# adaly/gridnext

Hardware: AMD Instinct MI355X
Metric: spots/sec training throughput (multimodal f+g) (higher is better)
Workload: dtype f32; 1 GPU; C4: multimodal f(DenseNet-121 @128px + count-MLP 2000 genes) + hex g on 78x64 Visium grids, 1 array (4992 spots) per GPU per step, f frozen/eval (tutorial mode), g trained with Adam, masked CE; spots_per_array=4992, parallelism=dp1

## Files before the change

### gridnext_amd/_lib.py

```python
import ctypes
import os

import torch

_HERE = os.path.dirname(os.path.abspath(__file__))
LIB_PATH = os.environ.get('GNX_LIB') or os.path.join(_HERE, 'libgridnext_hip.so')

_P, _I, _L, _F, _D = ctypes.c_void_p, ctypes.c_int, ctypes.c_long, ctypes.c_float, ctypes.c_double
_LL = ctypes.c_longlong

SIGNATURES = {
    'gnx_hexconv_fwd': (_I, [_P, _P, _P, _P, _P, _I, _I, _I, _I, _I, _I, _P]),
    'gnx_hexconv_bwd_data': (_I, [_P, _P, _P, _P, _I, _I, _I, _I, _I, _I, _P]),
    'gnx_hexconv_bwd_weight_workspace': (_L, [_I, _I, _I, _I, _I]),
    'gnx_hexconv_bwd_weight': (_I, [_P, _P, _P, _P, _P, _P, _I, _I, _I, _I, _I, _I, _I, _P]),
    'gnx_hexconv_bwd_weight_batch': (_I, [_P, _I, _P]),
    'gnx_hexconv_k_fwd': (_I, [_P, _P, _P, _P, _I, _I, _I, _I, _I, _I, _I, _P]),
    'gnx_hexconv_k_bwd_data': (_I, [_P, _P, _P, _I, _I, _I, _I, _I, _I, _I, _P]),
    'gnx_hexconv_k_bwd_weight_workspace': (_L, [_I, _I, _I, _I, _I, _I]),
    'gnx_hexconv_k_bwd_weight': (_I, [_P, _P, _P, _P, _P, _I, _I, _I, _I, _I, _I, _I, _I, _P]),
    'gnx_gridconv_fwd': (_I, [_P, _P, _P, _P, _I, _I, _I, _I, _I, _I, _I, _P]),
    'gnx_gridconv_bwd_data': (_I, [_P, _P, _P, _I, _I, _I, _I, _I, _I, _I, _P]),
    'gnx_gridconv_bwd_weight_workspace': (_L, [_I, _I, _I, _I, _I, _I, _I]),
    'gnx_gridconv_bwd_weight': (_I, [_P, _P, _P, _P, _P, _I, _I, _I, _I, _I, _I, _I, _I, _P]),
# ... 50 lines not shown
    'gnx_conv_stem_bnrelu_maxpool_h16': (_I, [_P, _P, _P, _L, _L, _I, _I, _I, _I, _I, _I, _I, _I, _P, _P, _P]),
    'gnx_conv_stem_bnrelu_maxpool_u8': (_I, [_P, _P, _P, _L, _L, _I, _I, _I, _I, _I, _I, _I, _I, _P, _P, _P, _I, _P]),
    'gnx_conv_stem_bnrelu_maxpool_f16mul': (_I, [_P, _I, _P, _P, _L, _L, _I, _I, _I, _I, _I, _I, _I, _I, _P, _P, _P, _P]),
    'gnx_u8_to_f32': (_I, [_P, _P, _L, _I, _I, _I, _P, _P]),
    'gnx_resize_ksize': (_I, [_I, _I]),
    'gnx_resize_crop_u8': (_I, [_P, _P, _L, _I, _I, _I, _I, _I, _I, _I, _I, _P, _P, _P, _P, _P]),
    'gnx_resize_crop_u8_f32': (_I, [_P, _P, _L, _I, _I, _I, _I, _I, _I, _I, _I, _P, _P, _P, _P, _P, _P]),
    'gnx_wsi_patch_grid_u8': (_I, [_P, _I, _I, _P, _I, _I, _I, _I, _I, _P, _P, _I, _P, _P]),
    'gnx_wsi_patch_grid_u8_f32': (_I, [_P, _I, _I, _P, _I, _I, _I, _I, _I, _P, _P, _I, _P, _P, _P]),
    'gnx_conv1x1_bnrelu_f16_h': (_I, [_P, _L, _P, _P, _L, _L, _I, _I, _P, _P, _P, _P, _I, _I, _P]),
    'gnx_conv1x1_bnrelu_h16': (_I, [_P, _L, _P, _P, _L, _L, _I, _I, _P, _P, _P, _P, _P]),
    'gnx_bnrelu_avgpool2_h16': (_I, [_P, _L, _P, _L, _L, _I, _I, _P, _P, _P]),
    'gnx_conv3x3_f16_dma_h': (_I, [_P, _L, _P, _P, _L, _L, _I, _I, _I, _P]),
    'gnx_bnrelu_avgpool_h16': (_I, [_P, _L, _P, _L, _L, _I, _I, _P, _P, _P]),
    'gnx_wgrad1x1_f16_workspace': (_L, [_L, _I, _I]),
    'gnx_wgrad1x1_f16': (_I, [_P, _L, _P, _L, _P, _P, _P, _P, _L, _I, _I, _P, _I, _P, _P]),
    'gnx_wgrad3x3_f16_workspace': (_L, [_L]),
    'gnx_wgrad3x3_f16': (_I, [_P, _L, _P, _P, _P, _L, _I, _P, _I, _P, _P]),
    'gnx_conv3x3_dgrad_bnrelu_bwd_f16_workspace': (_L, [_L]),
    'gnx_conv3x3_dgrad_bnrelu_bwd_f16': (_I, [_P, _L, _P, _P, _P, _L, _I, _P, _P, _P, _P, _P, _P, _P, _I, _P, _P]),
    'gnx_conv1x1_dgrad_bnrelu_bwd_f16_workspace': (_L, [_L, _I]),
    'gnx_conv1x1_dgrad_bnrelu_bwd_f16': (_I, [_P, _P, _P, _L, _P, _L, _L, _I, _P, _P, _P, _P, _P, _P, _P, _P, _I, _P, _P]),
    'gnx_conv1x1_dgrad_wgrad_f16_workspace': (_L, [_L, _I]),
    'gnx_conv1x1_dgrad_wgrad_bnrelu_bwd_f16': (_I, [_P, _P, _P, _L, _P, _L, _L, _I, _P, _P, _P, _P, _P, _P, _P, _P, _P, _I, _P, _P]),
    'gnx_tail_bwd_f16_workspace': (_L, [_L, _I]),
    'gnx_tail_bwd_f16': (_I, [_P, _L, _P, _L, _P, _L, _L, _I, _I, _P, _P, _P, _P, _P, _P, _P, _P, _I, _P, _P]),
    'gnx_trans_bwd_f16_workspace': (_L, [_L, _I, _I]),
    'gnx_trans_bwd_f16': (_I, [_P, _L, _P, _L, _P, _L, _L, _I, _I, _P, _P, _P, _P, _P, _P, _P, _P, _I, _P, _P]),
    'gnx_h16_cols_to_f32': (_I, [_P, _L, _P, _L, _L, _I, _P, _P, _P]),
    'gnx_stem_bwd_f16_workspace': (_L, [_L, _I]),
    'gnx_stem_bwd_f16': (_I, [_P, _P, _P, _P, _P, _P, _P, _L, _P, _P, _P, _P, _L, _I, _I, _P, _I, _P, _P]),
    'gnx_dense_layer_f16_pack': (_I, [_P, _P, _P, _P, _I, _P]),
    'gnx_dense_layer_f16': (_I, [_P, _L, _L, _I, _I, _P, _P, _P, _P, _P, _P, _P]),
    'gnx_dense_layer_f16_tape': (_I, [_P, _L, _L, _I, _I, _P, _P, _P, _P, _P, _P, _P, _L, _P]),
    'gnx_dense_bwd_f16_pack': (_I, [_P, _P, _P, _P, _I, _P]),
    'gnx_wgrad3x3_f16_lb': (_I, [_P, _L, _P, _L, _L, _P, _P, _L, _I, _P, _I, _P, _P]),
    'gnx_conv3x3_dgrad_bnrelu_bwd_f16_lb': (_I, [_P, _L, _P, _P, _L, _L, _P, _L, _I, _P, _P, _P, _P, _P, _P, _P, _I, _P, _P]),
    'gnx_conv3x3_bwd_f16_workspace': (_L, [_L]),
    'gnx_conv3x3_bwd_f16_lb': (_I, [_P, _L, _P, _P, _L, _L, _P, _P, _L, _I, _P, _P, _P, _P, _P, _P, _P, _I, _P, _P]),
    'gnx_conv1x1_dgrad_wgrad_bnrelu_bwd_f16_lb': (_I, [_P, _P, _P, _L, _L, _P, _L, _L, _L, _I, _P, _P, _P, _P, _P, _P, _P, _P, _P, _I,
                                                       _P, _P]),
    'gnx_tail_bwd_f16_lb': (_I, [_P, _L, _P, _L, _L, _P, _L, _L, _L, _I, _I, _P, _P, _P, _P, _P, _P, _P, _P, _I, _P, _P]),
    'gnx_trans_bwd_f16_lb': (_I, [_P, _L, _L, _P, _L, _L, _P, _L, _L, _L, _I, _I, _P, _P, _P, _P, _P, _P, _P, _P, _I, _P, _P]),
    'gnx_conv_stem_bnrelu_maxpool_f16mul_cb': (_I, [_P, _I, _P, _P, _L, _L, _I, _I, _I, _I, _I, _I, _I, _I, _P, _P, _P, _P]),
    'gnx_conv1x1_bnrelu_h16_cb': (_I, [_P, _L, _P, _P, _L, _L, _I, _I, _P, _P, _P, _P, _P]),
    'gnx_bnrelu_avgpool2_h16_cb': (_I, [_P, _L, _P, _L, _L, _I, _I, _P, _P, _P]),
    'gnx_transition_f16_pack': (_I, [_P, _P, _I, _I, _P]),
    'gnx_transition_f16': (_I, [_P, _L, _L, _I, _I, _I, _P, _P, _P, _P, _L, _P]),
    'gnx_transition_f16_tape': (_I, [_P, _L, _L, _I, _I, _I, _P, _P, _P, _P, _L, _P, _L, _P]),
    'gnx_bnrelu_avgpool_h16_cb': (_I, [_P, _L, _P, _L, _L, _I, _I, _P, _P, _P]),
    'gnx_conv3x3_bnrelu': (_I, [_P, _L, _P, _P, _L, _L, _I, _I, _I, _P, _P, _P]),
    'gnx_winograd_conv3x3_weights': (_I, [_P, _P, _I, _I, _P]),
    'gnx_conv3x3_winograd': (_I, [_P, _L, _P, _P, _L, _L, _I, _I, _I, _P]),
    'gnx_conv3x3_form': (_I, [_P, _L, _P, _P, _L, _L, _I, _I, _I, _P, _P, _P]),
    'gnx_conv3x3_winograd_form': (_I, [_P, _L, _P, _P, _L, _L, _I, _I, _I, _P]),
    'gnx_conv3x3_dgrad_bnrelu_bwd_form': (_I, [_P, _L, _P, _P, _L, _P, _L, _L, _I, _I, _I, _P, _P, _P, _P, _P, _P]),
    'gnx_conv3x3_f16_dma_form': (_I, [_P, _L, _P, _P, _L, _L, _I, _I, _I, _P]),
    'gnx_conv_stem': (_I, [_P, _P, _P, _L, _L, _I, _I, _I, _I, _I, _I, _I, _I, _P]),
    'gnx_conv_stem_bnrelu_maxpool': (_I, [_P, _P, _P, _L, _L, _I, _I, _I, _I, _I, _I, _I, _I, _P, _P, _P]),
    'gnx_conv_stem_bnrelu_maxpool_argmax': (_I, [_P, _P, _P, _L, _P, _L, _I, _I, _I, _I, _I, _I, _I, _I, _P, _P, _P]),
    'gnx_bnrelu_maxpool': (_I, [_P, _L, _P, _L, _L, _I, _I, _I, _P, _P, _P]),
    'gnx_bnrelu_avgpool': (_I, [_P, _L, _P, _L, _L, _I, _I, _P, _P, _P]),
    'gnx_spot_compact': (_I, [_P, _L, _L, _P, _P, _P, _P, _P]),
    'gnx_spot_broadcast_rows': (_I, [_P, _L, _L, _I, _P, _L, _P]),
    'gnx_conv_stem_bnrelu_maxpool_idx': (_I, [_P, _P, _P, _L, _L, _I, _I, _I, _I, _I, _I, _I, _I, _P, _P, _P, _L, _P]),
    'gnx_conv_stem_bnrelu_maxpool_u8_idx': (_I, [_P, _P, _P, _L, _L, _I, _I, _I, _I, _I, _I, _I, _I, _P, _P, _P, _P, _L, _P]),
    'gnx_bnrelu_avgpool_idx': (_I, [_P, _L, _P, _L, _L, _I, _I, _P, _P, _P, _L, _P]),
    'gnx_wgrad_workspace': (_L, [_L, _I, _I, _I]),
    'gnx_wgrad_bnrelu': (_I, [_P, _L, _P, _L, _P, _P, _P, _P, _L, _I, _I, _I, _I, _I, _I, _P]),
    'gnx_wgrad_bnrelu_batch': (_I, [_P, _I, _I, _P]),
    'gnx_transpose_weight': (_I, [_P, _P, _I, _I, _P]),
    'gnx_relayout_weights_batch': (_I, [_P, _I, _I, _P]),
    'gnx_repack_conv3x3_bwd': (_I, [_P, _P, _I, _I, _P]),
    'gnx_rows_broadcast': (_I, [_P, _L, _P, _L, _L, _I, _I, _F, _P]),
    'gnx_avgpool2_bwd': (_I, [_P, _L, _P, _L, _L, _I, _I, _P]),
    'gnx_maxpool_bwd': (_I, [_P, _L, _P, _L, _P, _L, _P, _L, _L, _I, _I, _I, _P, _P, _P]),
    'gnx_bnrelu_maxpool_argmax': (_I, [_P, _L, _P, _L, _P, _L, _I, _I, _I, _P, _P, _P]),
    'gnx_maxpool_bwd_argmax': (_I, [_P, _P, _L, _P, _L, _L, _I, _I, _I, _P]),
    'gnx_maxpool_bwd_argmax_bnrelu': (_I, [_P, _P, _L, _P, _L, _P, _P, _L, _L, _I, _I, _I, _P]),
    'gnx_conv0_wgrad_workspace': (_L, [_L, _I, _I, _I, _I, _I, _I, _I]),
    'gnx_conv0_wgrad': (_I, [_P, _P, _L, _P, _P, _L, _I, _I, _I, _I, _I, _I, _I, _I, _P]),
    'gnx_conv0_dgrad': (_I, [_P, _L, _P, _P, _L, _I, _I, _I, _I, _I, _I, _I, _P]),
    'gnx_softmax_rows': (_I, [_P, _L, _L, _I, _P, _L, _P, _P]),
    'gnx_gemm_f32': (_I, [_P, _L, _I, _P, _L, _I, _P, _P, _L, _L, _L, _L, _I, _P]),
    'gnx_gemm_f32_workspace': (_L, [_L, _L, _L]),
    'gnx_gemm_f32_ws': (_I, [_P, _L, _I, _P, _L, _I, _P, _P, _L, _L, _L, _L, _I, _P, _P]),
    'gnx_fingerprint128_split_bytes': (_L, []),
    'gnx_fingerprint128_batch_workspace': (_L, [ctypes.c_size_t, _I]),
    'gnx_fingerprint128_batch': (_I, [_P, ctypes.c_size_t, _I, _P, _P, _P]),
    'gnx_rgb_hist_u8_workspace': (_L, [ctypes.c_size_t]),
    'gnx_rgb_hist_u8': (_I, [_P, ctypes.c_size_t, _P, _P, _P]),
    'gnx_rgb_lut_u8': (_I, [_P, _P, ctypes.c_size_t, _P, _P]),
}

_lib = None
_ERRORS = {-1: 'bad argument', -2: 'kernel launch failed', -3: 'unsupported shape'}
ERR_UNSUPPORTED = -3


class HipExtensionMissing(RuntimeError):
    pass


def lib():
    global _lib
    if _lib is None:
# ... 45 lines not shown
```

### gridnext_amd/csrc/conv3x3.hip

```cpp
#include "fwd_common.h"

namespace {

constexpr int C3_BM = 128, C3_BN = 32;

__global__ __launch_bounds__(256) void conv3x3_kernel(const float* __restrict__ A, long lda,
                                                      const float* __restrict__ Wr, float* __restrict__ out, long ldc,
                                                      long M, int N, int K, int S, const float* __restrict__ scale,
                                                      const float* __restrict__ shift, int vecA, int vecW) {
    extern __shared__ __attribute__((aligned(16))) float lds[];
    const int strip = C3_BM + 2 * S + 2;
    float* As = lds;
    float* Bs = lds + strip * LDK;
    const int t = threadIdx.x, lane = t & 63, wave = t >> 6, h = lane >> 5, i = lane & 31;
    const long P0 = (long)blockIdx.x * C3_BM;
    const long base = P0 - S - 1;
    const int n0 = blockIdx.y * C3_BN;
    const bool has_act = scale != nullptr;

    const long P = P0 + 32 * wave + i;
    unsigned mask = 0;
    if (P < M) {
        const int rem = (int)(P % ((long)S * S));
        const int y = rem / S, x = rem - y * S;
// ... 439 lines not shown
        if constexpr (!NK1) store16(0, std::integral_constant<int, 0>{});
    }
    asm volatile("s_waitcnt vmcnt(0)" ::: "memory");
    if constexpr (BNADJ) {
#pragma unroll
        for (int ct = 0; ct < 4; ++ct) {
            const float sb = adj_b[ct] + __shfl_xor(adj_b[ct], 32), sg = adj_g[ct] + __shfl_xor(adj_g[ct], 32);
            if (h == 0) {
                float* sl = bn.slab + (long)(blockIdx.x * NW + wave) * 2 * N + 32 * ct + i;
                sl[0] = sb;
                sl[N] = sg;
            }
        }
    }
}

constexpr int C3_ADJ_LANES = 16;
__global__ __launch_bounds__(64 * C3_ADJ_LANES) void c3_adj_reduce_kernel(const float* __restrict__ slab, int nblk, int C,
                                                                          float* __restrict__ dbeta,
                                                                          float* __restrict__ dgamma, int accumulate) {
    __shared__ float part[C3_ADJ_LANES][64];
    const int cl = threadIdx.x & 63, rl = threadIdx.x >> 6;
    const int idx = blockIdx.x * 64 + cl;
    float s0 = 0.f;
    if (idx < 2 * C) {
        const int q = idx / C, c = idx - q * C;
        const int per = (nblk + C3_ADJ_LANES - 1) / C3_ADJ_LANES;
        int b = rl * per;
        const int be = b + per < nblk ? b + per : nblk;
        for (; b + 16 <= be; b += 16) {
            float v[16];
#pragma unroll
            for (int u = 0; u < 16; ++u) v[u] = slab[((long)(b + u) * 2 + q) * C + c];
#pragma unroll
            for (int u = 0; u < 16; ++u) s0 += v[u];
        }
        for (; b < be; ++b) s0 += slab[((long)b * 2 + q) * C + c];
    }
    part[rl][cl] = s0;
    __syncthreads();
    if (rl == 0 && idx < 2 * C) {
        const int q = idx / C, c = idx - q * C;
        float tot = 0.f;
#pragma unroll
        for (int u = 0; u < C3_ADJ_LANES; ++u) tot += part[u][cl];
        float* dst = q == 0 ? dbeta : dgamma;
        if (dst) dst[c] = accumulate ? dst[c] + tot : tot;
    }
}

#ifndef GNX_WINO_DBG
#define GNX_WINO_DBG 0
#endif
template <int S>
__global__ __launch_bounds__(256) void conv3x3_wino_kernel(const float* __restrict__ A, int lda,
                                                          const float* __restrict__ Wu, float* __restrict__ out,
                                                          int ldc, int M, int K) {
    constexpr int BM = 256, NPAIR = 128;
    constexpr int RAWN = BM + 2 * S + 2, SRAW = (RAWN + 15) & ~15;
    constexpr int NV = NPAIR + S, NVR = (NV + 15) & ~15;
    constexpr int RAWB = SRAW * 64, UB = 12 * 32 * 64, VB = NVR * 64;
    constexpr int OFF_RAW = 0, OFF_U = 2 * RAWB, OFF_V = OFF_U + 2 * UB, OFF_Z = OFF_V + 4 * VB;
    static_assert(OFF_Z + 1024 <= 160 * 1024, "LDS");
    constexpr int NPR = SRAW / 16, NPU = 24;
    constexpr int NSR = (NPR + 3) / 4, NSU = NPU / 4;
    static_assert(NSR + NSU <= 24, "one DMA slot per MFMA step");
    __shared__ __attribute__((aligned(16))) char lds[OFF_Z + 1024];
    const int t = threadIdx.x, lane = t & 63, h = lane >> 5, i = lane & 31;
    const int wave = __builtin_amdgcn_readfirstlane(t >> 6);
    for (int z = t; z < 256; z += 256) reinterpret_cast<float*>(lds + OFF_Z)[z] = 0.f;
    const int T = (M + BM - 1) / BM;
    const int nk2 = K >> 5;
    int G = gridDim.x;
    asm volatile("" : "+s"(G));
    const int bx = blockIdx.x;
    const int bid = (G & 7) == 0 ? (bx & 7) * (G >> 3) + (bx >> 3) : bx;
    auto tile_of = [&](int round) {
        const int base = round * G;
        return base + (base + G <= T ? bid : bx);
    };
    const unsigned lb = lds_addr(lds);

    const int pix = ((lane & 15) - (wave & 1)) & 15;
    const unsigned voffA = ((unsigned)pix * lda + 4 * (lane >> 4)) * 4u;
    const unsigned voffU = ((unsigned)(lane & 15) * K + 4 * (lane >> 4)) * 4u;
    int nround = 0, ntile = tile_of(0), nchunk = 0;
    const __amdgpu_buffer_rsrc_t rU = __builtin_amdgcn_make_buffer_rsrc(const_cast<float*>(Wu), 0, 12 * 32 * K * 4, 0x00020000);
    auto issue_slot = [&](auto slot_c, int buf) {
        constexpr int slot = decltype(slot_c)::value;
        if constexpr (slot < NSR) {
            const int p = wave + 4 * slot;
            if ((NPR % 4) && slot == NSR - 1 && p >= NPR) return;
            const int row0 = ntile * BM - S - 1 + 16 * p;
            char* d = lds + OFF_RAW + buf * RAWB + p * 1024;
            if (__builtin_expect(row0 >= 0 && row0 + 15 < M, 1)) {
                const __amdgpu_buffer_rsrc_t rs = __builtin_amdgcn_make_buffer_rsrc(
                    const_cast<float*>(A + (long)row0 * lda), 0, (15 * lda + K) * 4, 0x00020000);
                dma16_buf(rs, voffA, 64 * nchunk, lds_addr(d));
            } else {
                int Pr = row0 + pix;
                Pr = Pr < 0 ? 0 : (Pr >= M ? M - 1 : Pr);
                dma16_global(A + (long)Pr * lda + 16 * nchunk + 4 * (lane >> 4), lds_addr(d));
            }
        } else {
            const int p = wave + 4 * (slot - NSR);
            dma16_buf(rU, voffU, (16 * p * K + 16 * nchunk) * 4, lds_addr(lds + OFF_U + buf * UB + p * 1024));
        }
    };
    auto advance_next = [&]() {
        if (++nchunk == 2 * nk2) { nchunk = 0; ntile = tile_of(++nround); }
        if (ntile >= T) ntile = bid;
    };
    static_for<0, NSR + NSU>([&](auto sc) { issue_slot(sc, 0); });
    advance_next();

    constexpr int NIT = (NVR * 4 + 255) / 256;
    const int r = 32 * wave + i;
    const unsigned fU = lb + OFF_U + (i >> 4) * 1024 + (i & 15) * 16 + h * 256;

    bool stored = false;
    for (int round = 0, tile = tile_of(0); tile < T; tile = tile_of(++round)) {
        const int P = tile * BM + 2 * r;
        const int y = (P % (S * S)) / S;
        unsigned bV[12];
#pragma unroll
        for (int dy = 0; dy < 3; ++dy) {
            const int jp = r + S / 2 + (dy - 1) * (S / 2);
            const bool ok = (dy == 1) || (dy == 0 ? y > 0 : y < S - 1);
#pragma unroll
            for (int xi = 0; xi < 4; ++xi)
                bV[dy * 4 + xi] = ok ? lb + OFF_V + xi * VB + (jp >> 4) * 1024 + (jp & 15) * 16 + h * 256 : lb + OFF_Z;
        }
        f32x16 acc[4][2];
#pragma unroll
        for (int xi = 0; xi < 4; ++xi)
#pragma unroll
            for (int q = 0; q < 2; ++q)
#pragma unroll
                for (int e = 0; e < 16; ++e) acc[xi][q][e] = 0.f;

        auto do_chunk = [&](auto par_c) {
            constexpr int par = decltype(par_c)::value;
            if (stored) asm volatile("s_waitcnt vmcnt(32)" ::: "memory");
            else asm volatile("s_waitcnt vmcnt(0)" ::: "memory");
            stored = false;
            asm volatile("s_barrier" ::: "memory");
#if GNX_WINO_DBG != 1
            {
                const char* raw = lds + OFF_RAW + par * RAWB;
#pragma unroll
                for (int j = 0; j < NIT; ++j) {
                    const int it = t + 256 * j;
                    const int c = it / NVR, jp = it - c * NVR;
                    if (it < NVR * 4 && jp < NV) {
                        const int xin = (2 * jp) & (S - 1);
                        auto at = [&](int q) {
                            return raw + (q >> 4) * 1024 + c * 256 + (((q & 15) + ((q >> 4) & 1)) & 15) * 16;
                        };
                        const char* zr = lds + OFF_Z;
                        typedef float f2 __attribute__((ext_vector_type(2)));
                        struct F4 { f2 lo, hi; };
                        auto rd = [&](const char* p) { return *reinterpret_cast<const F4*>(p); };
                        const F4 d0 = rd(xin == 0 ? zr : at(2 * jp)), d1 = rd(at(2 * jp + 1)), d2 = rd(at(2 * jp + 2)),
                                 d3 = rd(xin + 2 == S ? zr : at(2 * jp + 3));
                        char* v = lds + OFF_V + (jp >> 4) * 1024 + c * 256 + (jp & 15) * 16;
                        *reinterpret_cast<F4*>(v) = F4{d0.lo - d2.lo, d0.hi - d2.hi};
                        *reinterpret_cast<F4*>(v + VB) = F4{d1.lo + d2.lo, d1.hi + d2.hi};
                        *reinterpret_cast<F4*>(v + 2 * VB) = F4{d2.lo - d1.lo, d2.hi - d1.hi};
                        *reinterpret_cast<F4*>(v + 3 * VB) = F4{d1.lo - d3.lo, d1.hi - d3.hi};
                    }
                }
            }
#endif
            asm volatile("s_waitcnt lgkmcnt(0)" ::: "memory");
            asm volatile("s_barrier" ::: "memory");
            const unsigned bU = fU + par * UB;
            auto rdA = [&](auto e_c) {
                constexpr int e = decltype(e_c)::value;
                return lds_read4<(e & 1) * 512>(bV[e >> 1]);
            };
            auto rdB = [&](auto e_c) {
                constexpr int e = decltype(e_c)::value;
                return lds_read4<(e >> 1) * 2048 + (e & 1) * 512>(bU);
            };
            f32x4 a = rdA(std::integral_constant<int, 0>{}), bq = rdB(std::integral_constant<int, 0>{});
            static_for<0, 24>([&](auto step_c) {
                constexpr int step = decltype(step_c)::value;
                constexpr int xi = (step >> 1) & 3;
                f32x4 na, nb;
                if constexpr (step < 23) {
                    na = rdA(std::integral_constant<int, step + 1>{});
                    nb = rdB(std::integral_constant<int, step + 1>{});
                    asm volatile("s_waitcnt lgkmcnt(2)" : "+v"(a), "+v"(bq));
                } else {
                    asm volatile("s_waitcnt lgkmcnt(0)" : "+v"(a), "+v"(bq));
                }
                acc[xi][0] = __builtin_amdgcn_mfma_f32_32x32x2f32(a[0], bq[0], acc[xi][0], 0, 0, 0);
                acc[xi][1] = __builtin_amdgcn_mfma_f32_32x32x2f32(a[1], bq[1], acc[xi][1], 0, 0, 0);
                acc[xi][0] = __builtin_amdgcn_mfma_f32_32x32x2f32(a[2], bq[2], acc[xi][0], 0, 0, 0);
                acc[xi][1] = __builtin_amdgcn_mfma_f32_32x32x2f32(a[3], bq[3], acc[xi][1], 0, 0, 0);
#if GNX_WINO_DBG != 2
                if constexpr (step < NSR + NSU) issue_slot(step_c, par ^ 1);
#endif
                if constexpr (step < 23) { a = na; bq = nb; }
            });
            advance_next();
        };
        for (int c2 = 0; c2 < nk2; ++c2) {
            do_chunk(std::integral_constant<int, 0>{});
            do_chunk(std::integral_constant<int, 1>{});
        }
        {
            const int left = M - tile * BM;
            const __amdgpu_buffer_rsrc_t ro = __builtin_amdgcn_make_buffer_rsrc(
                out + (long)tile * BM * ldc, 0, (left < BM ? left : BM) * ldc * 4, 0x00020000);
            const int vo = (2 * (32 * wave + 4 * h) * ldc + i) * 4;
#pragma unroll
            for (int e = 0; e < 16; ++e) {
                const float m0 = acc[0][0][e] + acc[0][1][e], m1 = acc[1][0][e] + acc[1][1][e];
                const float m2 = acc[2][0][e] + acc[2][1][e], m3 = acc[3][0][e] + acc[3][1][e];
                const int row = 2 * ((e & 3) + 8 * (e >> 2));
                __builtin_amdgcn_raw_buffer_store_b32(__float_as_uint((m0 + m1) + m2), ro, vo, row * ldc * 4, 0);
                __builtin_amdgcn_raw_buffer_store_b32(__float_as_uint((m1 - m2) - m3), ro, vo, (row + 1) * ldc * 4, 0);
            }
        }
        stored = true;
    }
    asm volatile("s_waitcnt vmcnt(0)" ::: "memory");
}

__global__ void winograd_weights_kernel(const float* __restrict__ w, float* __restrict__ wu, int N, int K) {
    const long idx = (long)blockIdx.x * blockDim.x + threadIdx.x;
    const long total = (long)3 * N * K;
    if (idx >= total) return;
    const int k = (int)(idx % K), n = (int)((idx / K) % N), dy = (int)(idx / ((long)K * N));
    const float* g = w + ((long)n * K + k) * 9 + dy * 3;
    const float g0 = g[0], g1 = g[1], g2 = g[2];
    const long nk = (long)N * K;
    float* u = wu + (long)dy * 4 * nk + (long)n * K + k;
    u[0] = g0;
    u[nk] = 0.5f * ((g0 + g2) + g1);
    u[2 * nk] = 0.5f * ((g0 + g2) - g1);
    u[3 * nk] = g2;
}

__global__ void repack3x3_kernel(const float* __restrict__ w, float* __restrict__ wr, int N, int K) {
    const long idx = (long)blockIdx.x * blockDim.x + threadIdx.x;
    const long total = (long)9 * N * K;
    if (idx >= total) return;
    const int k = (int)(idx % K), n = (int)((idx / K) % N), tap = (int)(idx / ((long)K * N));
    wr[idx] = w[((long)n * K + k) * 9 + tap];
}

struct C3Plan { int rc, form, wgs, wgy; };
enum { GNX_C3_GENERIC = 0, GNX_C3_PIPE5 = 1, GNX_C3_PIPE6 = 2, GNX_C3_PIPE7 = 3, GNX_C3_PIPE9 = 4, GNX_C3_DMA4 = 5, GNX_C3_DMA8 = 6,
       GNX_C3_DMAG4 = 7, GNX_C3_DMAG8 = 8, GNX_C3_WINO = 9 };

bool c3_dma_s(int S) {
    return S == 4 || S == 7 || S == 8 || S == 14 || S == 16 || S == 28 || S == 32 || S == 56 || S == 64;
}
bool c3_pow2_s(int S) { return S == 4 || S == 8 || S == 16 || S == 32 || S == 64; }
bool c3_eight_waves(long M, int S) { return S <= 32 && M % 256 == 0 && M / 256 >= 1024; }
int c3_persistent_wgs(long M, int bm) { return (int)(M / bm > 256 ? 256 : M / bm); }

size_t c3_lds_bytes(int S) { return ((size_t)(C3_BM + 2 * S + 2) * LDK + 9 * 32 * LDK + LDK) * sizeof(float); }

C3Plan conv3x3_plan(const float* A, long lda, const float* Wr, const float* out, long ldc, long M, int N, int K, int S,
                    const float* scale, const float* shift) {
    C3Plan p = {GNX_OK, GNX_C3_GENERIC, 0, 0};
    if (!A || !Wr || !out || M < 0 || N <= 0 || K <= 0 || S <= 0 || lda < K || ldc < N || (!scale) != (!shift) ||
        (M % ((long)S * S)) != 0) {
        p.rc = GNX_ERR_BAD_ARG;
        return p;
    }
    if (M == 0) return p;
    if (c3_lds_bytes(S) > 160 * 1024) {
        p.rc = GNX_ERR_UNSUPPORTED;
        return p;
    }
    const bool vecA = al16(A) && lda % 4 == 0 && K % 4 == 0 && (!scale || (al16(scale) && al16(shift)));
    const bool vecW = al16(Wr) && K % 4 == 0;
// ... 56 lines not shown
    else if (N != C3_BN || (K & 127) != 0 || (M % C3_BM) != 0 || (lda16 & 7) != 0 || !al16(A16) || !al16(Wr16) ||
             M * (lda16 > ldc ? lda16 : ldc) >= (1L << 31))
        p.rc = GNX_ERR_UNSUPPORTED;
    else if (M > 0) {
        if (!c3_pow2_s(S)) {
            p.rc = GNX_ERR_UNSUPPORTED;
            return p;
        }
        p.form = c3_eight_waves(M, S) ? 8 : 4;
        p.wgs = c3_persistent_wgs(M, 32 * p.form);
    }
    return p;
}

int c3_answer(const C3Plan& p, int* workgroups) {
    if (workgroups) *workgroups = p.rc == GNX_OK ? p.wgs : 0;
    return p.rc != GNX_OK ? p.rc : p.form;
}

}

GNX_EXPORT int gnx_conv3x3_form(const float* A, long lda, const float* Wr, const float* out, long ldc, long M, int N, int K,
                                int S, const float* scale, const float* shift, int* workgroups) {
    return c3_answer(conv3x3_plan(A, lda, Wr, out, ldc, M, N, K, S, scale, shift), workgroups);
}
GNX_EXPORT int gnx_conv3x3_winograd_form(const float* A, long lda, const float* Wu, const float* out, long ldc, long M, int N,
                                         int K, int S, int* workgroups) {
    return c3_answer(conv3x3_wino_plan(A, lda, Wu, out, ldc, M, N, K, S), workgroups);
}
GNX_EXPORT int gnx_conv3x3_dgrad_bnrelu_bwd_form(const float* dY, long lddy, const float* Wb, const float* A_act, long lda,
                                                 const float* dX, long lddx, long M, int N, int K, int S, const float* scale,
                                                 const float* shift, const float* mean, const float* invstd,
                                                 const float* workspace, int* workgroups) {
    return c3_answer(conv3x3_dgrad_bn_plan(dY, lddy, Wb, A_act, lda, dX, lddx, M, N, K, S, scale, shift, mean, invstd, workspace),
                     workgroups);
}
GNX_EXPORT int gnx_conv3x3_f16_dma_form(const void* A16, long lda16, const void* Wr16, const void* out, long ldc, long M, int N,
                                        int K, int S, int* workgroups) {
    return c3_answer(conv3x3_f16_plan(A16, lda16, Wr16, out, ldc, M, N, K, S), workgroups);
}

GNX_EXPORT int gnx_repack_conv3x3(const float* w, float* wr, int N, int K, hipStream_t stream) {
    if (!w || !wr || N <= 0 || K <= 0) return GNX_ERR_BAD_ARG;
    repack3x3_kernel<<<gnx_cdiv(9L * N * K, 256), 256, 0, stream>>>(w, wr, N, K);
    return gnx_launch_status();
}

GNX_EXPORT int gnx_winograd_conv3x3_weights(const float* w, float* wu, int N, int K, hipStream_t stream) {
    if (!w || !wu || N <= 0 || K <= 0) return GNX_ERR_BAD_ARG;
    winograd_weights_kernel<<<gnx_cdiv(3L * N * K, 256), 256, 0, stream>>>(w, wu, N, K);
    return gnx_launch_status();
}

GNX_EXPORT int gnx_conv3x3_winograd(const float* A, long lda, const float* Wu, float* out, long ldc, long M, int N, int K,
                                    int S, hipStream_t stream) {
    const C3Plan p = conv3x3_wino_plan(A, lda, Wu, out, ldc, M, N, K, S);
    if (p.rc != GNX_OK || p.wgs == 0) return p.rc;
#define GNX_WINO(SS)                                                                                        \
    conv3x3_wino_kernel<SS><<<p.wgs, 256, 0, stream>>>(A, (int)lda, Wu, out, (int)ldc, (int)M, K);           \
    return gnx_launch_status()
    switch (S) {
        case 4: GNX_WINO(4);
        case 8: GNX_WINO(8);
        case 16: GNX_WINO(16);
        case 32: GNX_WINO(32);
        case 64: GNX_WINO(64);
        default: return GNX_ERR_UNSUPPORTED;
    }
#undef GNX_WINO
}

GNX_EXPORT long gnx_conv3x3_dgrad_bn_workspace(long M, int N) { return 256L * 8 * 2 * N; }

GNX_EXPORT int gnx_conv3x3_dgrad_bnrelu_bwd(const float* dY, long lddy, const float* Wb, const float* A_act, long lda,
                                            float* dX, long lddx, long M, int N, int K, int S, const float* scale,
                                            const float* shift, const float* mean, const float* invstd, float* dgamma,
                                            float* dbeta, int accumulate, float* workspace, hipStream_t stream) {
    const C3Plan p = conv3x3_dgrad_bn_plan(dY, lddy, Wb, A_act, lda, dX, lddx, M, N, K, S, scale, shift, mean, invstd, workspace);
    if (p.rc != GNX_OK || p.wgs == 0) return p.rc;
    C3BnAdj bn = {A_act, (int)lda, scale, shift, mean, invstd, workspace};
    const int nblk = p.wgs * p.form;
#define GNX_DMAA(SS)                                                                                              \
    do {                                                                                                          \
        if constexpr (SS <= 32) {                                                                                 \
            if (p.form == 8) {                                                                                    \
                conv3x3_dma_kernel<SS, 8, 32, true, false, false, true><<<p.wgs, 512, 0, stream>>>(               \
                    dY, (int)lddy, Wb, dX, (int)lddx, (int)M, K, N, bn);                                          \
                break;                                                                                            \
            }                                                                                                     \
        }                                                                                                         \
        conv3x3_dma_kernel<SS, 4, 32, true, false, false, true><<<p.wgs, 256, 0, stream>>>(                       \
            dY, (int)lddy, Wb, dX, (int)lddx, (int)M, K, N, bn);                                                  \
    } while (0)
    switch (S) {
        case 4: GNX_DMAA(4); break;
        case 8: GNX_DMAA(8); break;
        case 16: GNX_DMAA(16); break;
        case 32: GNX_DMAA(32); break;
        case 64: GNX_DMAA(64); break;
        default: return GNX_ERR_UNSUPPORTED;
    }
#undef GNX_DMAA
    if (dgamma || dbeta)
        c3_adj_reduce_kernel<<<gnx_cdiv(2 * N, 64), 64 * C3_ADJ_LANES, 0, stream>>>(workspace, nblk, N, dbeta, dgamma, accumulate);
    return gnx_launch_status();
}

GNX_EXPORT int gnx_conv3x3_bnrelu(const float* A, long lda, const float* Wr, float* out, long ldc, long M, int N, int K,
                                  int S, const float* scale, const float* shift, hipStream_t stream) {
    const C3Plan p = conv3x3_plan(A, lda, Wr, out, ldc, M, N, K, S, scale, shift);
    if (p.rc != GNX_OK || p.wgs == 0) return p.rc;
    const size_t lds_bytes = c3_lds_bytes(S);
    static size_t configured = 0;
    if (lds_bytes > configured) {
        if (hipFuncSetAttribute(reinterpret_cast<const void*>(conv3x3_kernel), hipFuncAttributeMaxDynamicSharedMemorySize,
                                (int)lds_bytes) != hipSuccess)
            return GNX_ERR_LAUNCH;
        configured = lds_bytes;
    }
    const int vecA = al16(A) && lda % 4 == 0 && K % 4 == 0 && (!scale || (al16(scale) && al16(shift)));
    const int vecW = al16(Wr) && K % 4 == 0;
    const dim3 grid(p.wgs, p.wgy);
// ... 98 lines not shown
```

### include/gridnext_hip.h

```cpp
#ifndef GRIDNEXT_HIP_H
#define GRIDNEXT_HIP_H

#include <stddef.h>
#include <stdint.h>

#ifdef __cplusplus
extern "C" {
#endif

#define GNX_OK 0
#define GNX_ERR_BAD_ARG (-1)
#define GNX_ERR_LAUNCH (-2)
#define GNX_ERR_UNSUPPORTED (-3)

typedef void* gnx_stream_t;

int gnx_hexconv_fwd(const float* x, const float* kernel0, const float* kernel1, const float* bias, float* y,
                    int B, int H, int W, int I, int O, int mode, gnx_stream_t stream);
int gnx_hexconv_bwd_data(const float* dy, const float* kernel0, const float* kernel1, float* dx,
                         int B, int H, int W, int I, int O, int mode, gnx_stream_t stream);
long gnx_hexconv_bwd_weight_workspace(int B, int H, int W, int I, int O);
int gnx_hexconv_bwd_weight(const float* x, const float* dy, float* dkernel0, float* dkernel1, float* dbias,
                           float* workspace, int B, int H, int W, int I, int O, int mode, int accumulate,
                           gnx_stream_t stream);
// ... 100 lines not shown
int gnx_conv1x1_bnrelu_act(const float* A, long lda, const float* W, float* out, long ldc, long M, int N, int K,
                           const float* scale, const float* shift, const float* out_scale, const float* out_shift,
                           gnx_stream_t stream);
long gnx_conv1x1_split_pack_halves(int K);
int gnx_conv1x1_split_pack(const float* W, void* Wp, int K, gnx_stream_t stream);
int gnx_conv1x1_bnrelu_act_split(const float* A, long lda, const void* Wp, float* out, long ldc, long M, int K,
                                 const float* scale, const float* shift, const float* out_scale, const float* out_shift,
                                 gnx_stream_t stream);
long gnx_conv3x3_split_pack_halves(void);
int gnx_conv3x3_split_pack(const float* W, void* Wp, gnx_stream_t stream);
int gnx_conv3x3_split(const float* A, long lda, const void* Wp, float* out, long ldc, long M, int S, gnx_stream_t stream);
long gnx_wgrad1x1_split_workspace(long M, int N, int K);
int gnx_wgrad1x1_split(const float* dY, long lddy, const float* X, long ldx, const float* scale, const float* shift, float* dW,
                       float* workspace, long M, int N, int K, int accumulate, gnx_stream_t stream);
long gnx_wgrad3x3_split_workspace(long M);
int gnx_wgrad3x3_split(const float* dY, long lddy, const float* A, long lda, float* dW, float* workspace, long M, int S,
                       int accumulate, gnx_stream_t stream);
long gnx_conv1x1_dgrad_bn_workspace(long M, int N);
int gnx_conv1x1_dgrad_bnrelu_bwd(const float* dY, long lddy, const float* Wt, const float* X, long ldx, float* dX, long lddx,
                                 long M, int N, int K, const float* scale, const float* shift, const float* mean,
                                 const float* invstd, float* dgamma, float* dbeta, int accumulate, float* workspace,
                                 gnx_stream_t stream);
long gnx_conv1x1_dgrad_wgrad_workspace(long M, int K);
int gnx_conv1x1_dgrad_wgrad_bnrelu_bwd(const float* dB, long lddb, const float* W1t, const float* X, long ldx, float* G, long ldg,
                                       long M, int K, const float* scale, const float* shift, const float* mean,
                                       const float* invstd, float* dgamma, float* dbeta, float* dW, float* workspace,
                                       int accumulate, gnx_stream_t stream);
#define GNX_C1_GENERIC 0
#define GNX_C1_GENERIC_VEC 1
#define GNX_C1_POOL 2
#define GNX_C1_POOL_VEC 3
#define GNX_C1_SPLIT 4
#define GNX_C1_WS 5
#define GNX_C1_WS_ACT 6
#define GNX_C1_WS_POOL 7
int gnx_conv1x1_form(const float* A, long lda, const float* W, const float* out, long ldc, long M, int N, int K,
                     const float* scale, const float* shift, int pool, int S_in, const float* out_scale, const float* out_shift,
                     const float* workspace, int* workgroups, int* splits);
int gnx_conv1x1_dgrad_bnrelu_bwd_form(const float* dY, long lddy, const float* Wt, const float* X, long ldx, const float* dX,
                                      long lddx, long M, int N, int K, const float* scale, const float* shift, const float* mean,
                                      const float* invstd, const float* dgamma, const float* dbeta, int accumulate,
                                      const float* workspace, int* workgroups);
long gnx_conv3x3_dgrad_bn_workspace(long M, int N);
int gnx_conv3x3_dgrad_bnrelu_bwd(const float* dY, long lddy, const float* Wb, const float* A_act, long lda, float* dX,
                                 long lddx, long M, int N, int K, int S, const float* scale, const float* shift,
                                 const float* mean, const float* invstd, float* dgamma, float* dbeta, int accumulate,
                                 float* workspace, gnx_stream_t stream);
int gnx_repack_conv3x3(const float* w, float* wr, int N, int K, gnx_stream_t stream);
int gnx_conv3x3_bnrelu(const float* A, long lda, const float* Wr, float* out, long ldc, long M, int N, int K, int S,
                       const float* scale, const float* shift, gnx_stream_t stream);
int gnx_winograd_conv3x3_weights(const float* w, float* wu, int N, int K, gnx_stream_t stream);
int gnx_conv3x3_winograd(const float* A, long lda, const float* Wu, float* out, long ldc, long M, int N, int K, int S,
                         gnx_stream_t stream);
#define GNX_C3_GENERIC 0
#define GNX_C3_PIPE5 1
#define GNX_C3_PIPE6 2
#define GNX_C3_PIPE7 3
#define GNX_C3_PIPE9 4
#define GNX_C3_DMA4 5
#define GNX_C3_DMA8 6
#define GNX_C3_DMAG4 7
#define GNX_C3_DMAG8 8
#define GNX_C3_WINO 9
int gnx_conv3x3_form(const float* A, long lda, const float* Wr, const float* out, long ldc, long M, int N, int K, int S,
                     const float* scale, const float* shift, int* workgroups);
int gnx_conv3x3_winograd_form(const float* A, long lda, const float* Wu, const float* out, long ldc, long M, int N, int K, int S,
                              int* workgroups);
int gnx_conv3x3_dgrad_bnrelu_bwd_form(const float* dY, long lddy, const float* Wb, const float* A_act, long lda, const float* dX,
                                      long lddx, long M, int N, int K, int S, const float* scale, const float* shift,
                                      const float* mean, const float* invstd, const float* workspace, int* workgroups);
int gnx_conv3x3_f16_dma_form(const void* A16, long lda16, const void* Wr16, const void* out, long ldc, long M, int N, int K,
                             int S, int* workgroups);
int gnx_conv_stem(const float* x, const float* w, float* out, long ldc, long imgs, int Cin, int H, int W, int O,
                  int KH, int KW, int stride, int pad, gnx_stream_t stream);
int gnx_conv_stem_bnrelu_maxpool(const float* x, const float* w, float* out, long ldo, long imgs, int Cin, int H, int W,
                                 int O, int KH, int KW, int stride, int pad, const float* scale, const float* shift,
                                 gnx_stream_t stream);
int gnx_conv_stem_bnrelu_maxpool_argmax(const float* x, const float* w, float* out, long ldo, unsigned char* argmax,
                                        long imgs, int Cin, int H, int W, int O, int KH, int KW, int stride, int pad,
                                        const float* scale, const float* shift, gnx_stream_t stream);
int gnx_bnrelu_maxpool(const float* in, long ldi, float* out, long ldo, long imgs, int C, int Hi, int Wi,
                       const float* scale, const float* shift, gnx_stream_t stream);
int gnx_bnrelu_avgpool(const float* in, long ldi, float* out, long ldo, long imgs, int C, int S2,
                       const float* scale, const float* shift, gnx_stream_t stream);

int gnx_spot_compact(const void* x, long spot_bytes, long N, int* flags, int* fg_idx, int* bg_idx, int* counts,
                     gnx_stream_t stream);
int gnx_spot_broadcast_rows(float* rows, long ld, long n_rows, int C, const int* bg_idx, long n_bg, gnx_stream_t stream);
int gnx_conv_stem_bnrelu_maxpool_idx(const float* x, const float* w, float* out, long ldo, long imgs, int Cin, int H, int W,
                                     int O, int KH, int KW, int stride, int pad, const float* scale, const float* shift,
                                     const int* src_idx, long src_imgs, gnx_stream_t stream);
int gnx_conv_stem_bnrelu_maxpool_u8_idx(const unsigned char* x8, const float* w, float* out, long ldo, long imgs, int Cin,
                                        int H, int W, int O, int KH, int KW, int stride, int pad, const float* scale,
                                        const float* shift, const float* norm, const int* src_idx, long src_imgs,
                                        gnx_stream_t stream);
int gnx_bnrelu_avgpool_idx(const float* in, long ldi, float* out, long ldo, long imgs, int C, int S2, const float* scale,
                           const float* shift, const int* dst_idx, long dst_rows, gnx_stream_t stream);

int gnx_conv1x1_bnrelu_f16(const float* A, long lda, const float* W, float* out, long ldc, long M, int N, int K,
                           const float* scale, const float* shift, int pool, int S_in, gnx_stream_t stream);
int gnx_conv3x3_bnrelu_f16(const float* A, long lda, const float* Wr, float* out, long ldc, long M, int N, int K, int S,
                           const float* scale, const float* shift, gnx_stream_t stream);
int gnx_conv1x1_bnrelu_f16_act16(const float* A, long lda, const float* W, void* out16, long ldc16, long M, int N, int K,
                                 const float* scale, const float* shift, const float* out_scale, const float* out_shift,
                                 gnx_stream_t stream);
int gnx_conv3x3_f16_dma(const void* A16, long lda16, const void* Wr16, float* out, long ldc, long M, int N, int K, int S,
// ... 163 lines not shown
```

Measured before the change: 84360 spots/s.

## Compute Winograd input transform in registers instead of staging V tiles in LDS

Adds a register-path variant of the Winograd 3x3 conv kernel. It reads raw input rows straight from LDS with precomputed per-lane addresses, forms the input-transform differences in registers, and double-buffers the operand reads across MFMA groups. This removes the separate V-tile transform pass, its LDS storage and one barrier per chunk, and it becomes the default for the supported grid sizes. In exchange it uses more VGPRs, relies on hand-placed waitcnt/barrier ordering, and keeps the old LDS kernel available as a fallback entry point.

After: 85580 spots/s, median of 6. 1.01x the previous value.

```diff
diff --git a/gridnext_amd/_lib.py b/gridnext_amd/_lib.py
--- a/gridnext_amd/_lib.py
+++ b/gridnext_amd/_lib.py
@@ -126,6 +126,8 @@
     'gnx_conv3x3_bnrelu': (_I, [_P, _L, _P, _P, _L, _L, _I, _I, _I, _P, _P, _P]),
     'gnx_winograd_conv3x3_weights': (_I, [_P, _P, _I, _I, _P]),
     'gnx_conv3x3_winograd': (_I, [_P, _L, _P, _P, _L, _L, _I, _I, _I, _P]),
+    'gnx_conv3x3_winograd_lds': (_I, [_P, _L, _P, _P, _L, _L, _I, _I, _I, _P]),
+    'gnx_conv3x3_winograd_in_regs': (_I, [_I]),
     'gnx_conv3x3_form': (_I, [_P, _L, _P, _P, _L, _L, _I, _I, _I, _P, _P, _P]),
     'gnx_conv3x3_winograd_form': (_I, [_P, _L, _P, _P, _L, _L, _I, _I, _I, _P]),
     'gnx_conv3x3_dgrad_bnrelu_bwd_form': (_I, [_P, _L, _P, _P, _L, _P, _L, _L, _I, _I, _I, _P, _P, _P, _P, _P, _P]),
diff --git a/gridnext_amd/csrc/conv3x3.hip b/gridnext_amd/csrc/conv3x3.hip
--- a/gridnext_amd/csrc/conv3x3.hip
+++ b/gridnext_amd/csrc/conv3x3.hip
@@ -515,23 +515,31 @@
 #ifndef GNX_WINO_DBG
 #define GNX_WINO_DBG 0
 #endif
-template <int S>
-__global__ __launch_bounds__(256) void conv3x3_wino_kernel(const float* __restrict__ A, int lda,
-                                                          const float* __restrict__ Wu, float* __restrict__ out,
-                                                          int ldc, int M, int K) {
+template <int S, bool REG>
+__device__ __forceinline__ void conv3x3_wino_body(const float* __restrict__ A, int lda, const float* __restrict__ Wu,
+                                                  float* __restrict__ out, int ldc, int M, int K) {
     constexpr int BM = 256, NPAIR = 128;
     constexpr int RAWN = BM + 2 * S + 2, SRAW = (RAWN + 15) & ~15;
     constexpr int NV = NPAIR + S, NVR = (NV + 15) & ~15;
     constexpr int RAWB = SRAW * 64, UB = 12 * 32 * 64, VB = NVR * 64;
-    constexpr int OFF_RAW = 0, OFF_U = 2 * RAWB, OFF_V = OFF_U + 2 * UB, OFF_Z = OFF_V + 4 * VB;
-    static_assert(OFF_Z + 1024 <= 160 * 1024, "LDS");
+    constexpr int RAWS = RAWB + (REG ? 1024 : 0);
+    constexpr int OFF_RAW = 0, OFF_U = 2 * RAWS, OFF_V = OFF_U + 2 * UB, OFF_Z = OFF_V + 4 * VB;
+    constexpr int LDSB = REG ? OFF_V : OFF_Z + 1024;
+    static_assert(LDSB <= 160 * 1024, "LDS");
+    static_assert(RAWS + 512 < 65536 && UB + 11 * 2048 + 512 < 65536, "ds_read offset field");
     constexpr int NPR = SRAW / 16, NPU = 24;
     constexpr int NSR = (NPR + 3) / 4, NSU = NPU / 4;
-    static_assert(NSR + NSU <= 24, "one DMA slot per MFMA step");
-    __shared__ __attribute__((aligned(16))) char lds[OFF_Z + 1024];
+    static_assert(NSR + NSU <= (REG ? 20 : 24), "one DMA slot per MFMA step (REG: all ahead of the early barrier)");
+    __shared__ __attribute__((aligned(16))) char lds[LDSB];
     const int t = threadIdx.x, lane = t & 63, h = lane >> 5, i = lane & 31;
     const int wave = __builtin_amdgcn_readfirstlane(t >> 6);
-    for (int z = t; z < 256; z += 256) reinterpret_cast<float*>(lds + OFF_Z)[z] = 0.f;
+    if constexpr (REG) {
+        reinterpret_cast<float*>(lds + OFF_RAW + RAWB)[t] = 0.f;
+        reinterpret_cast<float*>(lds + OFF_RAW + RAWS + RAWB)[t] = 0.f;
+        asm volatile("s_waitcnt lgkmcnt(0)" ::: "memory");
+    } else {
+        for (int z = t; z < 256; z += 256) reinterpret_cast<float*>(lds + OFF_Z)[z] = 0.f;
+    }
     const int T = (M + BM - 1) / BM;
     const int nk2 = K >> 5;
     int G = gridDim.x;
@@ -555,7 +563,7 @@
             const int p = wave + 4 * slot;
             if ((NPR % 4) && slot == NSR - 1 && p >= NPR) return;
             const int row0 = ntile * BM - S - 1 + 16 * p;
-            char* d = lds + OFF_RAW + buf * RAWB + p * 1024;
+            char* d = lds + OFF_RAW + buf * RAWS + p * 1024;
             if (__builtin_expect(row0 >= 0 && row0 + 15 < M, 1)) {
                 const __amdgpu_buffer_rsrc_t rs = __builtin_amdgcn_make_buffer_rsrc(
                     const_cast<float*>(A + (long)row0 * lda), 0, (15 * lda + K) * 4, 0x00020000);
@@ -580,9 +588,21 @@
     constexpr int NIT = (NVR * 4 + 255) / 256;
     const int r = 32 * wave + i;
     const unsigned fU = lb + OFF_U + (i >> 4) * 1024 + (i & 15) * 16 + h * 256;
+    const unsigned zD = lb + OFF_RAW + RAWB + h * 256 + (i & 15) * 16;
+    unsigned relD[12];
+#pragma unroll
+    for (int dy = 0; dy < 3; ++dy)
+#pragma unroll
+        for (int j = 0; j < 4; ++j) {
+            const int q = 2 * (r + S / 2 + (dy - 1) * (S / 2)) + j, x = (2 * r) & (S - 1);
+            const bool pad = (j == 0 && x == 0) || (j == 3 && x == S - 2);
+            relD[dy * 4 + j] = pad ? zD : lb + OFF_RAW + (q >> 4) * 1024 + h * 256 + (((q & 15) + ((q >> 4) & 1)) & 15) * 16;
+        }
 
     bool stored = false;
+    f32x4 d[2][4], u[2][4];
     for (int round = 0, tile = tile_of(0); tile < T; tile = tile_of(++round)) {
+        bool primed = false;
         const int P = tile * BM + 2 * r;
         const int y = (P % (S * S)) / S;
         unsigned bV[12];
@@ -591,8 +611,10 @@
             const int jp = r + S / 2 + (dy - 1) * (S / 2);
             const bool ok = (dy == 1) || (dy == 0 ? y > 0 : y < S - 1);
 #pragma unroll
-            for (int xi = 0; xi < 4; ++xi)
-                bV[dy * 4 + xi] = ok ? lb + OFF_V + xi * VB + (jp >> 4) * 1024 + (jp & 15) * 16 + h * 256 : lb + OFF_Z;
+            for (int xi = 0; xi < 4; ++xi) {
+                if constexpr (REG) bV[dy * 4 + xi] = ok ? relD[dy * 4 + xi] : zD;
+                else bV[dy * 4 + xi] = ok ? lb + OFF_V + xi * VB + (jp >> 4) * 1024 + (jp & 15) * 16 + h * 256 : lb + OFF_Z;
+            }
         }
         f32x16 acc[4][2];
 #pragma unroll
@@ -602,15 +624,17 @@
 #pragma unroll
                 for (int e = 0; e < 16; ++e) acc[xi][q][e] = 0.f;
 
-        auto do_chunk = [&](auto par_c) {
-            constexpr int par = decltype(par_c)::value;
+        auto chunk_barrier = [&]() {
             if (stored) asm volatile("s_waitcnt vmcnt(32)" ::: "memory");
             else asm volatile("s_waitcnt vmcnt(0)" ::: "memory");
             stored = false;
             asm volatile("s_barrier" ::: "memory");
+        };
+        auto mul_lds = [&](auto par_c) {
+            constexpr int par = decltype(par_c)::value;
 #if GNX_WINO_DBG != 1
             {
-                const char* raw = lds + OFF_RAW + par * RAWB;
+                const char* raw = lds + OFF_RAW + par * RAWS;
 #pragma unroll
                 for (int j = 0; j < NIT; ++j) {
                     const int it = t + 256 * j;
@@ -667,11 +691,82 @@
 #endif
                 if constexpr (step < 23) { a = na; bq = nb; }
             });
+        };
+        auto mul_reg = [&](auto par_c, bool more) {
+            constexpr int par = decltype(par_c)::value;
+            auto rd = [&](auto buf_c, auto g_c) {
+                constexpr int buf = decltype(buf_c)::value, g = decltype(g_c)::value, dy = g >> 1, s2 = g & 1;
+                static_for<0, 4>([&](auto j_c) {
+                    constexpr int j = decltype(j_c)::value;
+                    d[g & 1][j] = lds_read4<buf * RAWS + s2 * 512>(bV[dy * 4 + j]);
+                });
+                static_for<0, 4>([&](auto xi_c) {
+                    constexpr int xi = decltype(xi_c)::value;
+                    u[g & 1][xi] = lds_read4<buf * UB + (dy * 4 + xi) * 2048 + s2 * 512>(fU);
+                });
+            };
+            if (!primed) {
+                chunk_barrier();
+                rd(par_c, std::integral_constant<int, 0>{});
+            }
+            static_for<0, 6>([&](auto g_c) {
+                constexpr int g = decltype(g_c)::value, b = g & 1;
+                if constexpr (g < 5) {
+                    rd(par_c, std::integral_constant<int, g + 1>{});
+                    asm volatile("s_waitcnt lgkmcnt(8)"
+                                 : "+v"(d[b][0]), "+v"(d[b][1]), "+v"(d[b][2]), "+v"(d[b][3]), "+v"(u[b][0]), "+v"(u[b][1]),
+                                   "+v"(u[b][2]), "+v"(u[b][3]));
+                } else {
+                    asm volatile("s_waitcnt lgkmcnt(0)"
+                                 : "+v"(d[b][0]), "+v"(d[b][1]), "+v"(d[b][2]), "+v"(d[b][3]), "+v"(u[b][0]), "+v"(u[b][1]),
+                                   "+v"(u[b][2]), "+v"(u[b][3]));
+                    if (more) {
+                        asm volatile("s_waitcnt vmcnt(0)" ::: "memory");
+                        asm volatile("s_barrier" ::: "memory");
+                        rd(std::integral_constant<int, par ^ 1>{}, std::integral_constant<int, 0>{});
+                    }
+                }
+                f32x2 dl[4] = {d[b][0].lo, d[b][1].lo, d[b][2].lo, d[b][3].lo};
+                f32x2 dh[4] = {d[b][0].hi, d[b][1].hi, d[b][2].hi, d[b][3].hi};
+                asm("" : "+v"(dl[0]), "+v"(dh[0]), "+v"(dl[1]), "+v"(dh[1]), "+v"(dl[2]), "+v"(dh[2]), "+v"(dl[3]), "+v"(dh[3]));
+                static_for<0, 4>([&](auto xi_c) {
+                    constexpr int xi = decltype(xi_c)::value;
+#if GNX_WINO_DBG == 1
+                    f32x2 lo = dl[xi], hi = dh[xi];
+#else
+                    constexpr int p = xi == 0 ? 0 : xi == 2 ? 2 : 1, q = xi == 0 ? 2 : xi == 2 ? 1 : xi == 1 ? 2 : 3;
+                    f32x2 lo = xi == 1 ? dl[p] + dl[q] : dl[p] - dl[q], hi = xi == 1 ? dh[p] + dh[q] : dh[p] - dh[q];
+                    asm("" : "+v"(lo), "+v"(hi));
+#endif
+                    const f32x4 w = u[b][xi];
+                    acc[xi][0] = __builtin_amdgcn_mfma_f32_32x32x2f32(lo[0], w[0], acc[xi][0], 0, 0, 0);
+                    acc[xi][1] = __builtin_amdgcn_mfma_f32_32x32x2f32(lo[1], w[1], acc[xi][1], 0, 0, 0);
+                    acc[xi][0] = __builtin_amdgcn_mfma_f32_32x32x2f32(hi[0], w[2], acc[xi][0], 0, 0, 0);
+                    acc[xi][1] = __builtin_amdgcn_mfma_f32_32x32x2f32(hi[1], w[3], acc[xi][1], 0, 0, 0);
+#if GNX_WINO_DBG != 2
+                    if constexpr (4 * g + xi < NSR + NSU) issue_slot(std::integral_constant<int, 4 * g + xi>{}, par ^ 1);
+#endif
+                    __builtin_amdgcn_sched_barrier(0);
+                });
+            });
+            if (more)
+                asm volatile("s_waitcnt lgkmcnt(0)"
+                             : "+v"(d[0][0]), "+v"(d[0][1]), "+v"(d[0][2]), "+v"(d[0][3]), "+v"(u[0][0]), "+v"(u[0][1]),
+                               "+v"(u[0][2]), "+v"(u[0][3]));
+            primed = more;
+        };
+        auto do_chunk = [&](auto par_c, bool more) {
+            if constexpr (REG) {
+                mul_reg(par_c, more);
+            } else {
+                chunk_barrier();
+                mul_lds(par_c);
+            }
             advance_next();
         };
         for (int c2 = 0; c2 < nk2; ++c2) {
-            do_chunk(std::integral_constant<int, 0>{});
-            do_chunk(std::integral_constant<int, 1>{});
+            do_chunk(std::integral_constant<int, 0>{}, true);
+            do_chunk(std::integral_constant<int, 1>{}, c2 + 1 < nk2);
         }
         {
             const int left = M - tile * BM;
@@ -690,6 +785,18 @@
         stored = true;
     }
     asm volatile("s_waitcnt vmcnt(0)" ::: "memory");
+}
+template <int S>
+__global__ __launch_bounds__(256) void conv3x3_wino_kernel(const float* __restrict__ A, int lda,
+                                                          const float* __restrict__ Wu, float* __restrict__ out,
+                                                          int ldc, int M, int K) {
+    conv3x3_wino_body<S, false>(A, lda, Wu, out, ldc, M, K);
+}
+template <int S>
+__global__ __launch_bounds__(256) void conv3x3_wino_reg_kernel(const float* __restrict__ A, int lda,
+                                                              const float* __restrict__ Wu, float* __restrict__ out,
+                                                              int ldc, int M, int K) {
+    conv3x3_wino_body<S, true>(A, lda, Wu, out, ldc, M, K);
 }
 
 __global__ void winograd_weights_kernel(const float* __restrict__ w, float* __restrict__ wu, int N, int K) {
@@ -852,12 +959,16 @@
     return gnx_launch_status();
 }
 
-GNX_EXPORT int gnx_conv3x3_winograd(const float* A, long lda, const float* Wu, float* out, long ldc, long M, int N, int K,
-                                    int S, hipStream_t stream) {
+namespace {
+bool c3_wino_reg_s(int S) { return S == 4 || S == 8 || S == 16 || S == 32 || S == 64; }
+
+int conv3x3_wino_launch(const float* A, long lda, const float* Wu, float* out, long ldc, long M, int N, int K, int S, bool reg,
+                        hipStream_t stream) {
     const C3Plan p = conv3x3_wino_plan(A, lda, Wu, out, ldc, M, N, K, S);
     if (p.rc != GNX_OK || p.wgs == 0) return p.rc;
-#define GNX_WINO(SS)                                                                                        \
-    conv3x3_wino_kernel<SS><<<p.wgs, 256, 0, stream>>>(A, (int)lda, Wu, out, (int)ldc, (int)M, K);           \
+#define GNX_WINO(SS)                                                                                                 \
+    if (reg) conv3x3_wino_reg_kernel<SS><<<p.wgs, 256, 0, stream>>>(A, (int)lda, Wu, out, (int)ldc, (int)M, K);      \
+    else conv3x3_wino_kernel<SS><<<p.wgs, 256, 0, stream>>>(A, (int)lda, Wu, out, (int)ldc, (int)M, K);              \
     return gnx_launch_status()
     switch (S) {
         case 4: GNX_WINO(4);
@@ -868,6 +979,16 @@
         default: return GNX_ERR_UNSUPPORTED;
     }
 #undef GNX_WINO
+}
+}
+GNX_EXPORT int gnx_conv3x3_winograd(const float* A, long lda, const float* Wu, float* out, long ldc, long M, int N, int K,
+                                    int S, hipStream_t stream) {
+    return conv3x3_wino_launch(A, lda, Wu, out, ldc, M, N, K, S, c3_wino_reg_s(S), stream);
+}
+GNX_EXPORT int gnx_conv3x3_winograd_in_regs(int S) { return c3_wino_reg_s(S) ? 1 : 0; }
+GNX_EXPORT int gnx_conv3x3_winograd_lds(const float* A, long lda, const float* Wu, float* out, long ldc, long M, int N, int K,
+                                        int S, hipStream_t stream) {
+    return conv3x3_wino_launch(A, lda, Wu, out, ldc, M, N, K, S, false, stream);
 }
 
 GNX_EXPORT long gnx_conv3x3_dgrad_bn_workspace(long M, int N) { return 256L * 8 * 2 * N; }
diff --git a/include/gridnext_hip.h b/include/gridnext_hip.h
--- a/include/gridnext_hip.h
+++ b/include/gridnext_hip.h
@@ -176,6 +176,9 @@
 int gnx_winograd_conv3x3_weights(const float* w, float* wu, int N, int K, gnx_stream_t stream);
 int gnx_conv3x3_winograd(const float* A, long lda, const float* Wu, float* out, long ldc, long M, int N, int K, int S,
                          gnx_stream_t stream);
+int gnx_conv3x3_winograd_in_regs(int S);
+int gnx_conv3x3_winograd_lds(const float* A, long lda, const float* Wu, float* out, long ldc, long M, int N, int K, int S,
+                             gnx_stream_t stream);
 #define GNX_C3_GENERIC 0
 #define GNX_C3_PIPE5 1
 #define GNX_C3_PIPE6 2
```
